# ccaven/tinyslam

Hardware: AMD Instinct MI355X
Metric: ORB extract throughput, 1280x720 (frames/sec; Mkeypoints/sec alongside) (higher is better)
Workload: dtype f32; 1 GPU; BASELINE.json configs[3]: batch of 256 independent 1280x720 RGBA frames per GPU, device-resident, full ORB (FAST-12 + orientation + blur + BRIEF-256); frames_per_gpu_per_batch=256, width=1280, height=720, hierarchy_depth=2, max_features=8192, content=default, mode=literal, input=rgba, pipeline=default, fp_contract=0, angle_bins=0, batches_in_flight=1, collate=none (1 GPU)

## Files before the change

tinyslam_amd/csrc/orb_api.hip:

```cpp
#include <hip/hip_runtime.h>
#include <chrono>
#include <cmath>

#include <cstdarg>
#include <cstdio>
#include <cstdlib>
#include <cstring>
#include <new>
#include <optional>
#include <string>
#include <algorithm>
#include <vector>

#include "../../include/tinyorb.h"
#include "orb_front_launch.h"
#include "orb_kernels_fused.h"
#include "orb_kernels_brief.h"
#include "orb_kernels_intended.h"
#include "orb_kernels_staged.h"
#include "orb_kernels_collate.h"
#include "orb_kernels_match.h"
#include "orb_kernels_verify.h"
#include "orb_kernels_epipolar.h"
#include "orb_kernels_guide.h"
// ... 146 lines not shown
    bool in_async[2] = {false, false};
    struct {
        bool single_memcpy = false, single_split = false, single_serial = false, single_sync = false, single_block = false;
        bool no_swizzle = false, quiet = false;
        bool front_generic = false, front_trace = false;
        int phase_mask = -1, brief_i_mask = -1, lds_pad = 0;
    } env;
    uint32_t* dv_count = nullptr;
    CornerData* dv_corners = nullptr;
    CornerDescriptor* dv_desc = nullptr;
    uint16_t* d_gray = nullptr;
    uint16_t* d_blur = nullptr;
    uint16_t* d_blur_rowc = nullptr;
    uint32_t blur_qa[kMaxLevels] = {0};
    uint32_t* d_counts = nullptr;
    CornerData* d_corners = nullptr;
    CornerDescriptor* d_desc = nullptr;
    uint32_t* out_counts[2] = {nullptr, nullptr};
    CornerData* out_corners[2] = {nullptr, nullptr};
    CornerDescriptor* out_desc[2] = {nullptr, nullptr};
    CornerData* d_seg = nullptr;
    uint32_t* d_seg_counts = nullptr;
    uint32_t* d_seg_before = nullptr;
    BandGeom bands{};
    RowsGeom rows{};
    BriefTGeom brieft{};
    bool use_brief_t = false;
    uint32_t band_rows_lvl[kMaxLevels] = {0};
    uint32_t ln_threads[kMaxLevels] = {0};
    uint32_t tile_w_lvl[kMaxLevels] = {0};
    uint32_t seg_classes = 1;
    uint32_t* d_pattern = nullptr;
    float* d_cos = nullptr;
    float* d_sin = nullptr;
    uint4* d_rot = nullptr;
    unsigned long long* d_stamps = nullptr;

    uint32_t* h_count = nullptr;
    uint32_t* d_single_done = nullptr;
    hipEvent_t single_done_ev = nullptr;
    uint32_t single_seq = 0;
    CornerData* h_corners = nullptr;
    CornerDescriptor* h_desc = nullptr;
    bool single_valid = false;

    uint32_t last_batch = 0;
// ... 375 lines not shown
}

bool brieft_geometry(const OrbProgram* p, const RowsGeom& rg, uint32_t n_classes, BriefTGeom* out) {
    BriefTGeom g{};
    g.n_slots = rg.n_slots;
    g.seg_cap = rg.seg_cap;
    g.n_classes = n_classes;
    uint32_t rows = 0;
    for (uint32_t m = 0; m < p->pyr.depth; m++) {
        g.flat_end[m] = rg.flat_end[m];
        g.qa[m] = rg.qa[m];
        g.row_base[m] = rows + (uint32_t)kBriefHalo;
        rows += p->pyr.h[m] + 2u * (uint32_t)kBriefHalo + 8u;
    }
    g.rows_padded = rows;
    g.oob = p->oob;
    *out = g;
    if (getenv("TINYORB_BRIEF_ROWS")) return false;
    return rg.n_slots >= 1u && rg.n_slots * n_classes <= kBriefTMaxSlots && rows <= kBriefTMaxRows;
}

int launch_brief(OrbProgram* p, hipStream_t s, uint32_t n, const RowsGeom& rows_geom, const uint16_t* d_blur,
                 const uint16_t* d_blur_rowc, const uint32_t* seg_counts, uint32_t* seg_before, const CornerData* seg,
                 uint32_t* d_counts, CornerData* d_corners, CornerDescriptor* d_desc) {
    const uint32_t cap = p->cfg.max_features;
    const BriefTables tab{p->d_pattern, p->d_cos, p->d_sin, p->d_rot};
    const bool use_t = p->use_brief_t;
    {
        LaunchScope ls(p, s, KID_PREFIX);
        hipLaunchKernelGGL(k_slot_prefix, dim3(n), dim3(64), 0, s, seg_counts, seg_before, d_counts, rows_geom.n_slots,
                           rows_geom.seg_cap, use_t ? p->brieft.n_classes : 1u);
    }
    if (use_t) {
        const BriefTGeom& tg = p->brieft;
        const dim3 grid(n, (cap + (uint32_t)kBriefNfChunk - 1u) / (uint32_t)kBriefNfChunk);
        {
            LaunchScope ls(p, s, KID_BRIEF_T);
#define BRIEF_T_LAUNCH(ROT_)                                                                                                         \
    hipLaunchKernelGGL((k_brief_t<kBriefTWaves, ROT_>), dim3(n, (cap + kBriefTThreads - 1u) / kBriefTThreads), dim3(kBriefTThreads), \
                       brieft_lds_bytes(tg), s, d_blur_rowc, p->pyr, tg, seg_counts, seg_before, seg, d_corners, cap, d_desc, tab)
            switch (rot_form(p->opt.fp_contract)) {
                case 1: BRIEF_T_LAUNCH(1); break;
                case 2: BRIEF_T_LAUNCH(2); break;
                default: BRIEF_T_LAUNCH(0); break;
            }
#undef BRIEF_T_LAUNCH
        }
        LaunchScope ls(p, s, KID_BRIEF_NF);
        if (p->oob != kOobZero)
            hipLaunchKernelGGL(k_brief_nf<true>, grid, dim3(256), 0, s, d_blur, d_blur_rowc, p->pyr, tg, seg_counts, seg_before, d_corners,
                               cap, d_desc, tab);
        else
            hipLaunchKernelGGL(k_brief_nf<false>, grid, dim3(256), 0, s, d_blur, d_blur_rowc, p->pyr, tg, seg_counts, seg_before, d_corners,
                               cap, d_desc, tab);
    } else {
        LaunchScope ls(p, s, KID_BRIEF_ROWS);
        RowsGeom rg = rows_geom;
        rg.oob = p->oob;
        rg.fp = p->opt.fp_contract;
        rg.split = 1u;
        while (rg.split < 16u && rg.n_slots * n * rg.split < 2048u) rg.split *= 2u;
        hipLaunchKernelGGL(k_brief_rows, dim3(rg.n_slots * rg.split, n), dim3(256), 0, s, d_blur, d_blur_rowc, p->pyr, rg,
                           seg_counts, seg_before, seg, d_corners, cap, d_desc, tab);
    }
    return ORB_OK;
}

FrontGeom fused_level_geometry(const OrbProgram* p, uint32_t lvl, uint32_t gw, uint32_t gh, uint32_t n) {
    const Pyramid& pyr = p->pyr;
    FrontGeom g = front_geometry(pyr, lvl, gw ? gw : 8u, gh, n, p->band_rows_lvl[lvl], p->tile_w_lvl[lvl], p->ln_threads[lvl]);
    if (gw == 0) g.gh = 0;
    g.slot_base = p->bands.slot_base[lvl];
    g.n_slots = p->bands.n_slots;
    g.seg_cap = p->bands.seg_cap;
    g.n_classes = p->seg_classes;
    g.stamps = p->d_stamps;
    if (p->env.phase_mask >= 0) g.phase_mask = (uint32_t)p->env.phase_mask;
// ... 51 lines not shown
            dim3 grid((pyr.w[lvl] + 63u) / 64u, (pyr.h[lvl] + 4u * kMipRows - 1u) / (4u * kMipRows), n);
            hipLaunchKernelGGL(k_mip, grid, dim3(64, 4), 0, sm, d_gray, pyr, lvl, (float)pyr.w[lvl - 1] / (float)pyr.w[lvl], (float)pyr.h[lvl - 1] / (float)pyr.h[lvl], p->wq);
        }
        const FrontGeom g = fused_level_geometry(p, lvl, gw, gh, n);
        hipStream_t s_lvl = s;
        if (g.n_bands * (g.tiled ? g.n_ct : 1u) != p->bands.slot_base[lvl + 1] - p->bands.slot_base[lvl])
            return fail(p, ORB_EINVAL, "internal: band count mismatch at level %u", lvl);
        if (!g.tiled && sizeof(BlurCol) * (size_t)g.n_var > 8u * (size_t)g.ts)
            return fail(p, ORB_EINVAL, "internal: blur column table of level %u does not fit", lvl);
        uint32_t lds = front_lds_bytes(g);
        lds += (uint32_t)p->env.lds_pad;
        if (lds > p->max_lds) return fail(p, ORB_EINVAL, "level %u needs %u bytes of LDS", lvl, lds);
        const dim3 grid(g.n_bands * (g.tiled ? g.n_ct : 1u) * n);
        FrontLaunch L{frames, p->frame_bytes, d_gray, d_blur, d_blur_rowc, pyr, g, p->threshold, d_seg_counts, d_seg, s_lvl, grid.x, lds,
                      p->band_rows_lvl[lvl], p->ln_threads[lvl], p->input_y8,
                      lvl == 0 && ((pyr.w[0] & 3u) || g.store_grey), p->oob != kOobZero, false};
        L.geo = front_pick_geo(p, L);
        {
            LaunchScope ls(p, s_lvl, lvl == 0 ? KID_FUSED_L0 : KID_FUSED_LN);
            const hipError_t e = kFrontLaunch[front_form(p->opt.fp_contract, lvl == 0 && !p->input_y8)](L);
            if (e != hipSuccess) return fail(p, ORB_EHIP, "k_front (level %u) failed to launch: %s", lvl, hipGetErrorString(e));
        }
    }
    if (with_brief) launch_brief(p, s, n, p->rows, d_blur, d_blur_rowc, d_seg_counts, d_seg_before, d_seg, d_counts, d_corners, d_desc);
    HIP_TRY(p, hipGetLastError());
    return ORB_OK;
}

int run_fused(OrbProgram* p, const uint8_t* frames, uint32_t n, hipStream_t s) {
    if (int rc = run_fused_range(p, frames, 0, n, s)) return rc;
    p->planes_valid = true;
    return ORB_OK;
}

uint32_t itile_width(uint32_t w) {
    const uint32_t w8 = (w + 7u) & ~7u;
    return w8 < (uint32_t)kITileW ? w8 : (uint32_t)kITileW;
}

bool fused_i_eligible(const OrbProgram* p) {
    if (!p->intended || (p->opt.flags & ORB_FLAG_STAGED)) return false;
    const Pyramid& pyr = p->pyr;
    if ((uint64_t)pyr.w[0] * pyr.h[0] > (1ull << 26)) return false;
    if ((pyr.w[0] & 3u) != 0u || pyr.w[0] < 8u) return false;
    return true;
}

// ... 514 lines not shown
    const size_t B = p->max_batch, cap = config->max_features;
    CREATE_TRY(hipMalloc(&p->d_gray, B * p->pyr.stride * sizeof(uint16_t)));
    CREATE_TRY(hipMalloc(&p->d_blur, B * p->pyr.stride * sizeof(uint16_t)));
    for (int set = 0; set < ((p->opt.flags & ORB_FLAG_DOUBLE_OUTPUT) ? 2 : 1); set++) {
        CREATE_TRY(hipMalloc(&p->out_counts[set], B * sizeof(uint32_t)));
        CREATE_TRY(hipMalloc(&p->out_corners[set], B * cap * sizeof(CornerData)));
        CREATE_TRY(hipMalloc(&p->out_desc[set], B * cap * sizeof(CornerDescriptor)));
        CREATE_TRY(hipMemset(p->out_counts[set], 0, B * sizeof(uint32_t)));
        CREATE_TRY(hipMemset(p->out_corners[set], 0, B * cap * sizeof(CornerData)));
        CREATE_TRY(hipMemset(p->out_desc[set], 0, B * cap * sizeof(CornerDescriptor)));
    }
    p->d_counts = p->out_counts[0];
    p->d_corners = p->out_corners[0];
    p->d_desc = p->out_desc[0];
    if (p->fused) {
        CREATE_TRY(hipMalloc(&p->d_blur_rowc, B * p->pyr.row_stride * sizeof(uint16_t)));
        CREATE_TRY(hipMemset(p->d_blur_rowc, 0, B * p->pyr.row_stride * sizeof(uint16_t)));
        const size_t lists = (size_t)p->bands.n_slots * p->seg_classes;
        CREATE_TRY(hipMalloc(&p->d_seg, B * lists * (size_t)p->bands.seg_cap * sizeof(CornerData)));
        CREATE_TRY(hipMalloc(&p->d_seg_counts, B * lists * sizeof(uint32_t)));
        CREATE_TRY(hipMemset(p->d_seg_counts, 0, B * lists * sizeof(uint32_t)));
        CREATE_TRY(hipMalloc(&p->d_seg_before, B * lists * sizeof(uint32_t)));
    }
    if (p->fused_x) {
        CREATE_TRY(hipMalloc(&p->d_blur_rowc, B * p->pyr.row_stride * sizeof(uint16_t)));
        CREATE_TRY(hipMemset(p->d_blur_rowc, 0, B * p->pyr.row_stride * sizeof(uint16_t)));
        CREATE_TRY(hipMalloc(&p->d_xband_counts, B * (size_t)p->xband_slots * sizeof(uint32_t)));
    }
    if (p->fused_i || p->fused_x) {
        const size_t n_seg = B * (size_t)p->itiles.n_slots;
        CREATE_TRY(hipMalloc(&p->d_iseg, n_seg * p->itiles.seg_cap * sizeof(CornerData)));
        CREATE_TRY(hipMalloc(&p->d_iseg_scores, n_seg * p->itiles.seg_cap * sizeof(float)));
        CREATE_TRY(hipMalloc(&p->d_iseg_counts, n_seg * sizeof(uint32_t)));
        CREATE_TRY(hipMemset(p->d_iseg_counts, 0, n_seg * sizeof(uint32_t)));
        CREATE_TRY(hipMalloc(&p->d_iseg_before, n_seg * sizeof(uint32_t)));
        CREATE_TRY(hipMalloc(&p->d_thr_key, B * sizeof(unsigned long long)));
    } else if (p->opt.flags & (ORB_FLAG_NMS | ORB_FLAG_INTENDED)) {
        uint32_t off = 0, width = W, height = H;
        for (uint32_t m = 0; m < p->pyr.depth; m++) {
            const uint32_t gw = ((width + 7u) / 8u) * 8u, gh = ((height + 7u) / 8u) * 8u;
            p->score_layout.off[m] = off;
            p->score_layout.pitch[m] = gw + 2u;
            off += (gw + 2u) * (gh + 2u);
            width /= 2u;
            height /= 2u;
        }
// ... 55 lines not shown
    if (!p) return;
    (void)hipSetDevice(p->device);
    if (p->stream) (void)hipStreamSynchronize(p->stream);
    for (auto& sp : p->pending) {
        (void)hipEventDestroy(sp.start);
        (void)hipEventDestroy(sp.stop);
    }
    for (auto e : p->event_pool) (void)hipEventDestroy(e);
    (void)hipFree(p->d_input);
    (void)hipFree(p->d_input_alt);
    for (hipEvent_t ev : p->in_uploaded)
        if (ev) (void)hipEventDestroy(ev);
    (void)hipFree(p->d_gray);
    (void)hipFree(p->d_blur);
    (void)hipFree(p->d_blur_rowc);
    for (int set = 0; set < 2; set++) {
        (void)hipFree(p->out_counts[set]);
        (void)hipFree(p->out_corners[set]);
        (void)hipFree(p->out_desc[set]);
    }
    (void)hipFree(p->d_seg);
    (void)hipFree(p->d_seg_counts);
    (void)hipFree(p->d_seg_before);
    (void)hipFree(p->d_score_planes);
    (void)hipFree(p->d_prov_counts);
    (void)hipFree(p->d_prov);
    (void)hipFree(p->d_prov_scores);
    (void)hipFree(p->d_xband_counts);
    (void)hipFree(p->d_iseg);
    (void)hipFree(p->d_iseg_scores);
    (void)hipFree(p->d_iseg_counts);
    (void)hipFree(p->d_iseg_before);
    (void)hipFree(p->d_thr_key);
    (void)hipFree(p->d_prov2_counts);
    (void)hipFree(p->d_prov2);
    (void)hipFree(p->d_prov2_scores);
    (void)hipFree(p->d_pattern);
    (void)hipFree(p->d_cos);
    (void)hipFree(p->d_sin);
    if (p->d_rot) (void)hipFree(p->d_rot);
    (void)hipFree(p->d_stamps);
    for (int st = 0; st < ST_COUNT; st++) {
        free_stage_buffers(p, st);
        if (p->stage[st].done) (void)hipEventDestroy(p->stage[st].done);
    }
    if (p->single_done_ev) (void)hipEventDestroy(p->single_done_ev);
// ... 1267 lines not shown
```

tinyslam_amd/csrc/orb_kernels_brief.h:

```cpp
#pragma once
#include "orb_kernels_fused.h"

namespace orb {

constexpr int kBriefTThreads = 256;
constexpr int kBriefTWaves = 6;
constexpr uint32_t kBriefTMaxSlots = 8192;
constexpr uint32_t kBriefTMaxRows = 12288;

struct BriefTGeom {
    uint32_t n_slots, seg_cap;
    uint32_t n_classes;
    uint32_t flat_end[kMaxLevels];
    uint32_t qa[kMaxLevels];
    uint32_t row_base[kMaxLevels];
    uint32_t rows_padded;
    uint32_t oob;
};

__host__ __device__ inline uint32_t brieft_lds_bytes(const BriefTGeom& g) {
    return (g.n_slots * g.n_classes + 1u) * 4u + ((g.rows_padded + 1u) & ~1u) * 2u;
}

__device__ __forceinline__ constexpr int pat_ax(int j) { return ORB_BRIEF_PATTERN[4 * j + 0]; }
__device__ __forceinline__ constexpr int pat_ay(int j) { return ORB_BRIEF_PATTERN[4 * j + 1]; }
__device__ __forceinline__ constexpr int pat_bx(int j) { return ORB_BRIEF_PATTERN[4 * j + 2]; }
__device__ __forceinline__ constexpr int pat_by(int j) { return ORB_BRIEF_PATTERN[4 * j + 3]; }

__device__ __forceinline__ uint32_t wave_inclusive_sum(uint32_t x) {
    int v = (int)x;
    v += __builtin_amdgcn_update_dpp(0, v, 0x111, 0xf, 0xf, true);
// ... 5 lines not shown
    return (uint32_t)v;
}

__device__ __forceinline__ void store_host_u32(uint32_t* p, uint32_t v) { *p = v; }
__device__ __forceinline__ void store_host_16(void* p, uint4 v) { *reinterpret_cast<uint4*>(p) = v; }

__device__ __forceinline__ uint32_t push_gt(uint32_t word, uint32_t a, uint32_t b) {
    return __builtin_amdgcn_alignbit(word, b - a, 31);
}

__device__ __forceinline__ void brief_t_stage_rows(uint16_t* rows, const uint16_t* __restrict__ src, const Pyramid& pyr,
                                                   const BriefTGeom& bg, uint32_t tid, uint32_t n_threads = kBriefTThreads) {
    uint32_t m = 0;
    for (uint32_t i = tid; i < bg.rows_padded; i += n_threads) {
        while (m + 1u < pyr.depth && i + (uint32_t)kBriefHalo >= bg.row_base[m + 1u]) m++;
        const uint32_t y = i - bg.row_base[m];
        uint16_t v = 0;
        if (y < pyr.h[m]) v = src[pyr.row_off[m] + y];
        else if (bg.oob != kOobZero) v = src[pyr.row_off[m] + (uint32_t)oob_index((int)y, (int)pyr.h[m], bg.oob)];
        rows[i] = v;
    }
}

template <int CHUNK = kBriefTThreads, bool STAGED = false, int ROT = 0>
__device__ __forceinline__ void brief_t_body(uint8_t* lds_raw, uint32_t frame, uint32_t chunk, const uint16_t* __restrict__ blur_rowc,
                                             const Pyramid& pyr, const BriefTGeom& bg, const uint32_t* __restrict__ seg_counts,
                                             const uint32_t* __restrict__ seg_before, const CornerData* __restrict__ segments,
                                             CornerData* __restrict__ corners, uint32_t cap,
                                             CornerDescriptor* __restrict__ descriptors, const BriefTables& tab,
                                             CornerData* __restrict__ host_corners = nullptr,
                                             CornerDescriptor* __restrict__ host_descriptors = nullptr) {
    const uint32_t n_ent = bg.n_slots * bg.n_classes;
    uint32_t* const before = reinterpret_cast<uint32_t*>(lds_raw);
    uint16_t* const rows = reinterpret_cast<uint16_t*>(before + n_ent + 1u);
    __shared__ uint32_t lv[kMaxLevels][2];

    const uint32_t tid = threadIdx.x;
    const size_t sbase = (size_t)frame * n_ent;
    uint32_t stored_total;
    if (STAGED) {
        if (tid < pyr.depth) lv[tid][0] = bg.flat_end[tid], lv[tid][1] = bg.row_base[tid];
        __syncthreads();
        stored_total = before[n_ent];
    } else {
        stored_total = seg_before[sbase + n_ent - 1u] + min(seg_counts[sbase + n_ent - 1u], bg.seg_cap);
    }
    const uint32_t n_frame = min(stored_total, cap);
    const uint32_t k0 = chunk * (uint32_t)CHUNK;
    if (k0 >= n_frame) return;

    if (!STAGED) {
        for (uint32_t s = tid; s < n_ent; s += kBriefTThreads) before[s] = seg_before[sbase + s];
        if (tid == 0) before[n_ent] = stored_total;
        if (tid < pyr.depth) lv[tid][0] = bg.flat_end[tid], lv[tid][1] = bg.row_base[tid];
        brief_t_stage_rows(rows, blur_rowc + (size_t)frame * pyr.row_stride, pyr, bg, tid);
        __syncthreads();
    }

    const uint32_t k = k0 + tid;
    if (tid >= (uint32_t)CHUNK || k >= n_frame) return;
    uint32_t lo = 0, hi = n_ent;
    while (hi - lo > 1u) {
        const uint32_t mid = (lo + hi) >> 1;
        if (before[mid] <= k)
            lo = mid;
        else
            hi = mid;
    }
    const uint32_t cls = lo >= bg.n_slots ? 1u : 0u, slot = lo - cls * bg.n_slots;
    const uint4 rec = *reinterpret_cast<const uint4*>(
        &segments[(((size_t)frame * bg.n_slots + slot) * bg.n_classes + cls) * bg.seg_cap + (k - before[lo])]);
    *reinterpret_cast<uint4*>(&corners[(size_t)frame * cap + k]) = rec;
    if (host_corners) store_host_16(&host_corners[k], rec);
    const uint32_t lvl = min(rec.w, pyr.depth - 1u);
    if (!(rec.x >= (uint32_t)kBriefHalo && rec.x < lv[lvl][0])) return;

    uint32_t d[8];
    uint4* const o = reinterpret_cast<uint4*>(descriptors + (size_t)frame * cap + k);
    if (bg.n_classes == 2u && k0 + (tid & ~63u) + 64u <= before[bg.n_slots]) {
        const uint16_t* base0 = rows + lv[lvl][1] + rec.y - kBriefHalo;
#pragma unroll
        for (int wd = 0; wd < 8; wd++) {
            uint32_t acc = 0;
#pragma unroll
            for (int i = 31; i >= 0; i--) {
                const int j = wd * 32 + i;
                acc = push_gt(acc, base0[pat_ay(j) + kBriefHalo], base0[pat_by(j) + kBriefHalo]);
            }
            d[wd] = acc;
        }
        o[0] = make_uint4(d[0], d[1], d[2], d[3]);
        o[1] = make_uint4(d[4], d[5], d[6], d[7]);
        if (host_descriptors) {
            store_host_16(reinterpret_cast<uint4*>(host_descriptors + k), make_uint4(d[0], d[1], d[2], d[3]));
            store_host_16(reinterpret_cast<uint4*>(host_descriptors + k) + 1, make_uint4(d[4], d[5], d[6], d[7]));
        }
        return;
    }
// ... 18 lines not shown
            } else {
                const float a2 = nstw * (float)pat_ax(j), a3 = ctw * (float)pat_ay(j);
                const float b2 = nstw * (float)pat_bx(j), b3 = ctw * (float)pat_by(j);
                ray = a2 + a3, rby = b2 + b3;
            }
            acc = push_gt(acc, base[(int)ray], base[(int)rby]);
        }
        d[wd] = acc;
    }
    o[0] = make_uint4(d[0], d[1], d[2], d[3]);
    o[1] = make_uint4(d[4], d[5], d[6], d[7]);
    if (host_descriptors) {
        store_host_16(reinterpret_cast<uint4*>(host_descriptors + k), make_uint4(d[0], d[1], d[2], d[3]));
        store_host_16(reinterpret_cast<uint4*>(host_descriptors + k) + 1, make_uint4(d[4], d[5], d[6], d[7]));
    }
}

template <int kWavesPerSimd, int ROT = 0>
__global__ __launch_bounds__(kBriefTThreads, kWavesPerSimd) void k_brief_t(const uint16_t* __restrict__ blur_rowc, Pyramid pyr, BriefTGeom bg,
                                                                const uint32_t* __restrict__ seg_counts,
                                                                const uint32_t* __restrict__ seg_before,
                                                                const CornerData* __restrict__ segments,
                                                                CornerData* __restrict__ corners, uint32_t cap,
                                                                CornerDescriptor* __restrict__ descriptors, BriefTables tab) {
    extern __shared__ __attribute__((aligned(16))) uint8_t lds_raw[];
    brief_t_body<kBriefTThreads, false, ROT>(lds_raw, blockIdx.x, blockIdx.y, blur_rowc, pyr, bg, seg_counts, seg_before, segments, corners, cap, descriptors, tab);
}

constexpr int kNfPatchCols = 48, kNfPatchRows = 2 * kBriefHalo + 1;
constexpr int kNfPatchHalfs = kNfPatchRows * kNfPatchCols;

__global__ __launch_bounds__(64) void k_rot_table(const uint32_t* __restrict__ pattern, const float* __restrict__ cos_tab,
                                                  const float* __restrict__ sin_tab, int pitch, int intended, uint4* __restrict__ out,
                                                  uint32_t fp = 0u, uint32_t angle_bins = 0u) {
    const uint32_t code = angle_bins ? (blockIdx.x * 6284u + 3142u) / angle_bins : blockIdx.x, lane = threadIdx.x;
    const float ct = cos_tab[code], st = sin_tab[code], nst = -st;
    uint32_t w[4];
#pragma unroll
    for (int e = 0; e < 4; e++) {
        const uint32_t pk = pattern[64u * (uint32_t)e + lane];
        const float pax = (float)(int8_t)(pk & 255u), pay = (float)(int8_t)((pk >> 8) & 255u);
        const float pbx = (float)(int8_t)((pk >> 16) & 255u), pby = (float)(int8_t)(pk >> 24);
        float rax, ray, rbx, rby;
        if (intended) {
            const float a0 = ct * pax, a1 = nst * pay, a2 = st * pax, a3 = ct * pay;
            const float b0 = ct * pbx, b1 = nst * pby, b2 = st * pbx, b3 = ct * pby;
            rax = a0 + a1, ray = a2 + a3, rbx = b0 + b1, rby = b2 + b3;
        } else {
            rotate_fp(ct, st, nst, pax, pay, rot_form(fp), &rax, &ray);
// ... 46 lines not shown
    __syncthreads();
    uint32_t start = 0, n_nf = 0;
#pragma unroll
    for (uint32_t w2 = 0; w2 < 4u; w2++) {
        if (w2 < wave) start += wave_n[w2];
        n_nf += wave_n[w2];
    }
    if (mine) list[start + (uint32_t)__popcll(m & ((1ull << lane) - 1ull))] = (uint16_t)tid;
    __syncthreads();
    if (wave >= n_nf) return;

    uint32_t* out_desc = reinterpret_cast<uint32_t*>(descriptors + (size_t)frame * cap + k0);
    uint16_t* const patch = patches[wave];
    for (uint32_t i = wave; i < n_nf; i += (uint32_t)NW) {
        const uint32_t idx = __builtin_amdgcn_readfirstlane((uint32_t)list[i]);
        uint4 r = recs[idx];
        r.x = __builtin_amdgcn_readfirstlane(r.x), r.y = __builtin_amdgcn_readfirstlane(r.y);
        r.z = __builtin_amdgcn_readfirstlane(r.z), r.w = __builtin_amdgcn_readfirstlane(r.w);
        const uint32_t lvl = min(r.w, pyr.depth - 1u);
        const int w = (int)__builtin_amdgcn_readfirstlane(lv[lvl][0]), h = (int)__builtin_amdgcn_readfirstlane(lv[lvl][1]);
        const int qa = (int)__builtin_amdgcn_readfirstlane(lv[lvl][2]);
        const uint16_t* rowc = blur_rowc + (size_t)frame * pyr.row_stride + __builtin_amdgcn_readfirstlane(lv[lvl][3]);
        const uint16_t* plane = blur + (size_t)frame * pyr.stride + __builtin_amdgcn_readfirstlane(lv[lvl][4]);
        const uint4 tt = tab.rot[(size_t)min(r.z, (uint32_t)(ORB_ANGLE_STEPS - 1)) * 64u + lane];
        const uint32_t tw[4] = {tt.x, tt.y, tt.z, tt.w};
        uint64_t bal[4];
        if ((w & 1) == 0) {
            const int c0 = ((int)r.x - kBriefHalo) & ~7;
            constexpr int kPiecesPerRow = kNfPatchCols / 8, kPieces = kNfPatchRows * kPiecesPerRow;
            constexpr int kRounds = (kPieces + 63) / 64;
            uint4 tv[kRounds];
            uint32_t rcv[kRounds];
            int kind[kRounds], where[kRounds];
#pragma unroll
            for (int rr = 0; rr < kRounds; rr++) {
                const int p = (int)lane + 64 * rr;
                const int pr = (int)(((float)p + 0.5f) * (1.0f / (float)kPiecesPerRow));
                const int pc = p - pr * kPiecesPerRow;
                const int gy0 = (int)r.y - kBriefHalo + pr, cx = c0 + 8 * pc;
                const int gy = OOB ? oob_index(gy0, h, bg.oob) : gy0;
                const bool in = p < kPieces && gy >= 0 && gy < h && cx >= 0 && cx < w;
                kind[rr] = !in ? 0 : (cx < qa ? 1 : (cx + 8 <= w ? 2 : 3));
                where[rr] = p < kPieces ? pr * kNfPatchCols + 8 * pc : -1;
                rcv[rr] = rowc[min(max(gy, 0), h - 1)];
                if (OOB && p < kPieces && !(cx >= 0 && cx < w)) {
                    const int xm = oob_index(cx, w, bg.oob);
                    if (xm >= qa) rcv[rr] = plane[(size_t)(uint32_t)(__mul24(gy, w) + xm)];
                    kind[rr] = 1;
                }
                tv[rr] = *reinterpret_cast<const uint4*>(plane + (kind[rr] == 2 ? (size_t)(uint32_t)(__mul24(gy, w) + cx) : (size_t)0));
            }
#pragma unroll
            for (int rr = 0; rr < kRounds; rr++) {
                uint4 v = make_uint4(0u, 0u, 0u, 0u);
                if (kind[rr] == 1) {
                    const uint32_t c2 = rcv[rr] | (rcv[rr] << 16);
                    v = make_uint4(c2, c2, c2, c2);
                } else if (kind[rr] == 2) {
                    v = tv[rr];
                } else if (kind[rr] == 3) {
                    const int p = (int)lane + 64 * rr;
                    const int pr = (int)(((float)p + 0.5f) * (1.0f / (float)kPiecesPerRow));
                    const int gy0 = (int)r.y - kBriefHalo + pr, cx = c0 + 8 * (p - pr * kPiecesPerRow);
                    const int gy = OOB ? oob_index(gy0, h, bg.oob) : gy0;
                    const uint16_t* src = plane + (size_t)(uint32_t)(__mul24(gy, w) + cx);
                    uint32_t t[8];
#pragma unroll
                    for (int q = 0; q < 8; q++) t[q] = cx + q < w ? (uint32_t)src[q] : (OOB ? (uint32_t)src[w - 1 - cx] : 0u);
                    v = make_uint4(t[0] | (t[1] << 16), t[2] | (t[3] << 16), t[4] | (t[5] << 16), t[6] | (t[7] << 16));
                }
                if (where[rr] >= 0) *reinterpret_cast<uint4*>(&patch[where[rr]]) = v;
            }
            __builtin_amdgcn_fence(__ATOMIC_RELEASE, "wavefront");
            __builtin_amdgcn_wave_barrier();
            const int xo = (int)r.x - c0;
            const uint8_t* const centre = reinterpret_cast<const uint8_t*>(patch + kBriefHalo * kNfPatchCols + xo);
#pragma unroll
            for (int e = 0; e < 4; e++) {
                const uint32_t va = *reinterpret_cast<const uint16_t*>(centre + rot_a(tw[e]));
                const uint32_t vb = *reinterpret_cast<const uint16_t*>(centre + rot_b(tw[e]));
                bal[e] = __ballot(va > vb);
            }
            __builtin_amdgcn_fence(__ATOMIC_RELEASE, "wavefront");
            __builtin_amdgcn_wave_barrier();
        } else {
            const int gy = (int)r.y - kBriefHalo + (int)lane;
            const uint32_t rowv = (gy >= 0 && gy < h && lane < 37u) ? (uint32_t)rowc[gy] : 0u;
#pragma unroll
            for (int e = 0; e < 4; e++) {
                const int oa = rot_a(tw[e]) >> 1, ob = rot_b(tw[e]) >> 1;
                const int dya = (oa + kNfPatchCols / 2 + 64 * kNfPatchCols) / kNfPatchCols - 64, dxa = oa - dya * kNfPatchCols;
                const int dyb = (ob + kNfPatchCols / 2 + 64 * kNfPatchCols) / kNfPatchCols - 64, dxb = ob - dyb * kNfPatchCols;
                const int xa = (int)r.x + dxa, ya = (int)r.y + dya;
                const int xb = (int)r.x + dxb, yb = (int)r.y + dyb;
                uint32_t va = (uint32_t)__shfl((int)rowv, dya + kBriefHalo);
                uint32_t vb = (uint32_t)__shfl((int)rowv, dyb + kBriefHalo);
                const bool ina = xa >= 0 && xa < w && ya >= 0 && ya < h;
                const bool inb = xb >= 0 && xb < w && yb >= 0 && yb < h;
                if (!ina)
                    va = OOB ? blur_sample_mapped(plane, rowc, w, h, qa, xa, ya, bg.oob) : 0u;
                else if (xa >= qa)
                    va = plane[(size_t)(uint32_t)(__mul24(ya, w) + xa)];
                if (!inb)
                    vb = OOB ? blur_sample_mapped(plane, rowc, w, h, qa, xb, yb, bg.oob) : 0u;
                else if (xb >= qa)
                    vb = plane[(size_t)(uint32_t)(__mul24(yb, w) + xb)];
                bal[e] = __ballot(va > vb);
            }
        }
        if (lane < 8u) {
            const uint64_t src = lane < 2u ? bal[0] : (lane < 4u ? bal[1] : (lane < 6u ? bal[2] : bal[3]));
            out_desc[(size_t)idx * 8u + lane] = (uint32_t)(src >> ((lane & 1u) * 32u));
            if (host_descriptors) store_host_u32(reinterpret_cast<uint32_t*>(host_descriptors + k0) + (size_t)idx * 8u + lane, (uint32_t)(src >> ((lane & 1u) * 32u)));
        }
    }
}

constexpr int kBriefNfChunk = 64;
template <bool OOB = false>
__global__ __launch_bounds__(256) void k_brief_nf(const uint16_t* __restrict__ blur, const uint16_t* __restrict__ blur_rowc,
                                                  Pyramid pyr, BriefTGeom bg, const uint32_t* __restrict__ seg_counts,
                                                  const uint32_t* __restrict__ seg_before,
                                                  const CornerData* __restrict__ corners, uint32_t cap,
                                                  CornerDescriptor* __restrict__ descriptors, BriefTables tab) {
    brief_nf_body<kBriefNfChunk, 4, OOB>(blockIdx.x, blockIdx.y, ~0u, blur, blur_rowc, pyr, bg, seg_counts, seg_before, corners, cap, descriptors, tab);
}

constexpr int kBriefOneChunk = 64;
constexpr int kSingleCountWords = 32, kSingleDoneWord = 16;
constexpr int kBriefOneThreads = 512;
template <int ROT = 0>
__global__ __launch_bounds__(kBriefOneThreads) void k_brief_one(const uint16_t* __restrict__ blur, const uint16_t* __restrict__ blur_rowc, Pyramid pyr,
                                                   BriefTGeom bg, const uint32_t* __restrict__ seg_counts,
                                                   uint32_t* __restrict__ seg_before, const CornerData* __restrict__ segments,
                                                   uint32_t* __restrict__ counts, CornerData* __restrict__ corners, uint32_t cap,
                                                   CornerDescriptor* __restrict__ descriptors, BriefTables tab,
                                                   uint32_t* __restrict__ host_count, CornerData* __restrict__ host_corners,
                                                   CornerDescriptor* __restrict__ host_descriptors, uint32_t* __restrict__ done_count,
                                                   uint32_t seq) {
    extern __shared__ __attribute__((aligned(16))) uint8_t lds_raw[];
    const uint32_t tid = threadIdx.x, chunk = blockIdx.x;
    const uint32_t n_ent = bg.n_slots * bg.n_classes;
#ifdef TINYORB_STAMPS
    uint64_t st[6];
    int n_st = 0;
#define BRIEF_ONE_STAMP() do { if (n_st < 6) st[n_st++] = wall_clock64(); } while (0)
#else
#define BRIEF_ONE_STAMP() do { } while (0)
// ... 60 lines not shown
```

Before: 544,900 frames/s.

## Pass non-flat keypoint bitmask from BRIEF-T kernel to skip empty NF blocks

The tiled BRIEF kernel now writes a per-64-keypoint ballot mask marking which keypoints fell outside the flat (row-cached) path. The follow-up non-flat BRIEF kernel reads this mask and exits immediately for chunks with no work, instead of recomputing segment prefix lookups and classifying every keypoint itself. It also specialises level-parameter lookup for two-level pyramids, avoiding the LDS table and barrier. This adds a small global mask buffer, an extra write per wave, and a dependency between the two kernels on the mask contents.

```diff
diff --git a/tinyslam_amd/csrc/orb_api.hip b/tinyslam_amd/csrc/orb_api.hip
--- a/tinyslam_amd/csrc/orb_api.hip
+++ b/tinyslam_amd/csrc/orb_api.hip
@@ -192,6 +192,7 @@
     CornerData* d_seg = nullptr;
     uint32_t* d_seg_counts = nullptr;
     uint32_t* d_seg_before = nullptr;
+    uint64_t* d_nf_mask[2] = {nullptr, nullptr};
     BandGeom bands{};
     RowsGeom rows{};
     BriefTGeom brieft{};
@@ -613,7 +614,7 @@
 
 int launch_brief(OrbProgram* p, hipStream_t s, uint32_t n, const RowsGeom& rows_geom, const uint16_t* d_blur,
                  const uint16_t* d_blur_rowc, const uint32_t* seg_counts, uint32_t* seg_before, const CornerData* seg,
-                 uint32_t* d_counts, CornerData* d_corners, CornerDescriptor* d_desc) {
+                 uint32_t* d_counts, CornerData* d_corners, CornerDescriptor* d_desc, uint32_t f0 = 0) {
     const uint32_t cap = p->cfg.max_features;
     const BriefTables tab{p->d_pattern, p->d_cos, p->d_sin, p->d_rot};
     const bool use_t = p->use_brief_t;
@@ -625,11 +626,13 @@
     if (use_t) {
         const BriefTGeom& tg = p->brieft;
         const dim3 grid(n, (cap + (uint32_t)kBriefNfChunk - 1u) / (uint32_t)kBriefNfChunk);
+        const uint32_t mask_words = brief_mask_words(cap);
+        uint64_t* const nf_mask = p->d_nf_mask[p->cur_set] + (size_t)f0 * mask_words;
         {
             LaunchScope ls(p, s, KID_BRIEF_T);
 #define BRIEF_T_LAUNCH(ROT_)                                                                                                         \
     hipLaunchKernelGGL((k_brief_t<kBriefTWaves, ROT_>), dim3(n, (cap + kBriefTThreads - 1u) / kBriefTThreads), dim3(kBriefTThreads), \
-                       brieft_lds_bytes(tg), s, d_blur_rowc, p->pyr, tg, seg_counts, seg_before, seg, d_corners, cap, d_desc, tab)
+                       brieft_lds_bytes(tg), s, d_blur_rowc, p->pyr, tg, seg_counts, seg_before, seg, d_corners, cap, d_desc, tab, nf_mask, mask_words)
             switch (rot_form(p->opt.fp_contract)) {
                 case 1: BRIEF_T_LAUNCH(1); break;
                 case 2: BRIEF_T_LAUNCH(2); break;
@@ -638,12 +641,16 @@
 #undef BRIEF_T_LAUNCH
         }
         LaunchScope ls(p, s, KID_BRIEF_NF);
-        if (p->oob != kOobZero)
-            hipLaunchKernelGGL(k_brief_nf<true>, grid, dim3(256), 0, s, d_blur, d_blur_rowc, p->pyr, tg, seg_counts, seg_before, d_corners,
-                               cap, d_desc, tab);
-        else
-            hipLaunchKernelGGL(k_brief_nf<false>, grid, dim3(256), 0, s, d_blur, d_blur_rowc, p->pyr, tg, seg_counts, seg_before, d_corners,
-                               cap, d_desc, tab);
+#define BRIEF_NF_LAUNCH(OOB_, TABLE_)                                                                                                  \
+    hipLaunchKernelGGL((k_brief_nf<OOB_, TABLE_>), grid, dim3(256), 0, s, d_blur, d_blur_rowc, p->pyr, tg, d_corners, cap, d_desc, tab, \
+                       nf_mask, mask_words)
+        const bool table = p->pyr.depth > 2u;
+        if (p->oob != kOobZero) {
+            if (table) BRIEF_NF_LAUNCH(true, true); else BRIEF_NF_LAUNCH(true, false);
+        } else {
+            if (table) BRIEF_NF_LAUNCH(false, true); else BRIEF_NF_LAUNCH(false, false);
+        }
+#undef BRIEF_NF_LAUNCH
     } else {
         LaunchScope ls(p, s, KID_BRIEF_ROWS);
         RowsGeom rg = rows_geom;
@@ -741,7 +748,7 @@
             if (e != hipSuccess) return fail(p, ORB_EHIP, "k_front (level %u) failed to launch: %s", lvl, hipGetErrorString(e));
         }
     }
-    if (with_brief) launch_brief(p, s, n, p->rows, d_blur, d_blur_rowc, d_seg_counts, d_seg_before, d_seg, d_counts, d_corners, d_desc);
+    if (with_brief) launch_brief(p, s, n, p->rows, d_blur, d_blur_rowc, d_seg_counts, d_seg_before, d_seg, d_counts, d_corners, d_desc, f0);
     HIP_TRY(p, hipGetLastError());
     return ORB_OK;
 }
@@ -1302,6 +1309,10 @@
         CREATE_TRY(hipMemset(p->d_seg_counts, 0, B * lists * sizeof(uint32_t)));
         CREATE_TRY(hipMalloc(&p->d_seg_before, B * lists * sizeof(uint32_t)));
     }
+    if (p->use_brief_t)
+        for (int set = 0; set < ((p->opt.flags & ORB_FLAG_DOUBLE_OUTPUT) ? 2 : 1); set++) {
+            CREATE_TRY(hipMalloc(&p->d_nf_mask[set], B * brief_mask_words((uint32_t)cap) * sizeof(uint64_t)));
+        }
     if (p->fused_x) {
         CREATE_TRY(hipMalloc(&p->d_blur_rowc, B * p->pyr.row_stride * sizeof(uint16_t)));
         CREATE_TRY(hipMemset(p->d_blur_rowc, 0, B * p->pyr.row_stride * sizeof(uint16_t)));
@@ -1403,6 +1414,7 @@
     (void)hipFree(p->d_seg);
     (void)hipFree(p->d_seg_counts);
     (void)hipFree(p->d_seg_before);
+    for (int set = 0; set < 2; set++) (void)hipFree(p->d_nf_mask[set]);
     (void)hipFree(p->d_score_planes);
     (void)hipFree(p->d_prov_counts);
     (void)hipFree(p->d_prov);
diff --git a/tinyslam_amd/csrc/orb_brief_nf_keypoint.inc b/tinyslam_amd/csrc/orb_brief_nf_keypoint.inc
--- /dev/null
+++ b/tinyslam_amd/csrc/orb_brief_nf_keypoint.inc
@@ -0,0 +1,91 @@
+        const uint4 tt = tab.rot[(size_t)min(r.z, (uint32_t)(ORB_ANGLE_STEPS - 1)) * 64u + lane];
+        const uint32_t tw[4] = {tt.x, tt.y, tt.z, tt.w};
+        uint64_t bal[4];
+        if ((w & 1) == 0) {
+            const int c0 = ((int)r.x - kBriefHalo) & ~7;
+            constexpr int kPiecesPerRow = kNfPatchCols / 8, kPieces = kNfPatchRows * kPiecesPerRow;
+            constexpr int kRounds = (kPieces + 63) / 64;
+            uint4 tv[kRounds];
+            uint32_t rcv[kRounds];
+            int kind[kRounds], where[kRounds];
+#pragma unroll
+            for (int rr = 0; rr < kRounds; rr++) {
+                const int p = (int)lane + 64 * rr;
+                const int pr = (int)(((float)p + 0.5f) * (1.0f / (float)kPiecesPerRow));
+                const int pc = p - pr * kPiecesPerRow;
+                const int gy0 = (int)r.y - kBriefHalo + pr, cx = c0 + 8 * pc;
+                const int gy = OOB ? oob_index(gy0, h, bg.oob) : gy0;
+                const bool in = p < kPieces && gy >= 0 && gy < h && cx >= 0 && cx < w;
+                kind[rr] = !in ? 0 : (cx < qa ? 1 : (cx + 8 <= w ? 2 : 3));
+                where[rr] = p < kPieces ? pr * kNfPatchCols + 8 * pc : -1;
+                rcv[rr] = rowc[min(max(gy, 0), h - 1)];
+                if (OOB && p < kPieces && !(cx >= 0 && cx < w)) {
+                    const int xm = oob_index(cx, w, bg.oob);
+                    if (xm >= qa) rcv[rr] = plane[(size_t)(uint32_t)(__mul24(gy, w) + xm)];
+                    kind[rr] = 1;
+                }
+                tv[rr] = *reinterpret_cast<const uint4*>(plane + (kind[rr] == 2 ? (size_t)(uint32_t)(__mul24(gy, w) + cx) : (size_t)0));
+            }
+#pragma unroll
+            for (int rr = 0; rr < kRounds; rr++) {
+                uint4 v = make_uint4(0u, 0u, 0u, 0u);
+                if (kind[rr] == 1) {
+                    const uint32_t c2 = rcv[rr] | (rcv[rr] << 16);
+                    v = make_uint4(c2, c2, c2, c2);
+                } else if (kind[rr] == 2) {
+                    v = tv[rr];
+                } else if (kind[rr] == 3) {
+                    const int p = (int)lane + 64 * rr;
+                    const int pr = (int)(((float)p + 0.5f) * (1.0f / (float)kPiecesPerRow));
+                    const int gy0 = (int)r.y - kBriefHalo + pr, cx = c0 + 8 * (p - pr * kPiecesPerRow);
+                    const int gy = OOB ? oob_index(gy0, h, bg.oob) : gy0;
+                    const uint16_t* src = plane + (size_t)(uint32_t)(__mul24(gy, w) + cx);
+                    uint32_t t[8];
+#pragma unroll
+                    for (int q = 0; q < 8; q++) t[q] = cx + q < w ? (uint32_t)src[q] : (OOB ? (uint32_t)src[w - 1 - cx] : 0u);
+                    v = make_uint4(t[0] | (t[1] << 16), t[2] | (t[3] << 16), t[4] | (t[5] << 16), t[6] | (t[7] << 16));
+                }
+                if (where[rr] >= 0) *reinterpret_cast<uint4*>(&patch[where[rr]]) = v;
+            }
+            __builtin_amdgcn_fence(__ATOMIC_RELEASE, "wavefront");
+            __builtin_amdgcn_wave_barrier();
+            const int xo = (int)r.x - c0;
+            const uint8_t* const centre = reinterpret_cast<const uint8_t*>(patch + kBriefHalo * kNfPatchCols + xo);
+#pragma unroll
+            for (int e = 0; e < 4; e++) {
+                const uint32_t va = *reinterpret_cast<const uint16_t*>(centre + rot_a(tw[e]));
+                const uint32_t vb = *reinterpret_cast<const uint16_t*>(centre + rot_b(tw[e]));
+                bal[e] = __ballot(va > vb);
+            }
+            __builtin_amdgcn_fence(__ATOMIC_RELEASE, "wavefront");
+            __builtin_amdgcn_wave_barrier();
+        } else {
+            const int gy = (int)r.y - kBriefHalo + (int)lane;
+            const uint32_t rowv = (gy >= 0 && gy < h && lane < 37u) ? (uint32_t)rowc[gy] : 0u;
+#pragma unroll
+            for (int e = 0; e < 4; e++) {
+                const int oa = rot_a(tw[e]) >> 1, ob = rot_b(tw[e]) >> 1;
+                const int dya = (oa + kNfPatchCols / 2 + 64 * kNfPatchCols) / kNfPatchCols - 64, dxa = oa - dya * kNfPatchCols;
+                const int dyb = (ob + kNfPatchCols / 2 + 64 * kNfPatchCols) / kNfPatchCols - 64, dxb = ob - dyb * kNfPatchCols;
+                const int xa = (int)r.x + dxa, ya = (int)r.y + dya;
+                const int xb = (int)r.x + dxb, yb = (int)r.y + dyb;
+                uint32_t va = (uint32_t)__shfl((int)rowv, dya + kBriefHalo);
+                uint32_t vb = (uint32_t)__shfl((int)rowv, dyb + kBriefHalo);
+                const bool ina = xa >= 0 && xa < w && ya >= 0 && ya < h;
+                const bool inb = xb >= 0 && xb < w && yb >= 0 && yb < h;
+                if (!ina)
+                    va = OOB ? blur_sample_mapped(plane, rowc, w, h, qa, xa, ya, bg.oob) : 0u;
+                else if (xa >= qa)
+                    va = plane[(size_t)(uint32_t)(__mul24(ya, w) + xa)];
+                if (!inb)
+                    vb = OOB ? blur_sample_mapped(plane, rowc, w, h, qa, xb, yb, bg.oob) : 0u;
+                else if (xb >= qa)
+                    vb = plane[(size_t)(uint32_t)(__mul24(yb, w) + xb)];
+                bal[e] = __ballot(va > vb);
+            }
+        }
+        if (lane < 8u) {
+            const uint64_t src = lane < 2u ? bal[0] : (lane < 4u ? bal[1] : (lane < 6u ? bal[2] : bal[3]));
+            out_desc[(size_t)idx * 8u + lane] = (uint32_t)(src >> ((lane & 1u) * 32u));
+            if (host_descriptors) store_host_u32(reinterpret_cast<uint32_t*>(host_descriptors + k0) + (size_t)idx * 8u + lane, (uint32_t)(src >> ((lane & 1u) * 32u)));
+        }
diff --git a/tinyslam_amd/csrc/orb_kernels_brief.h b/tinyslam_amd/csrc/orb_kernels_brief.h
--- a/tinyslam_amd/csrc/orb_kernels_brief.h
+++ b/tinyslam_amd/csrc/orb_kernels_brief.h
@@ -7,6 +7,7 @@
 constexpr int kBriefTWaves = 6;
 constexpr uint32_t kBriefTMaxSlots = 8192;
 constexpr uint32_t kBriefTMaxRows = 12288;
+__host__ __device__ inline uint32_t brief_mask_words(uint32_t cap) { return 4u * ((cap + (uint32_t)kBriefTThreads - 1u) / (uint32_t)kBriefTThreads); }
 
 struct BriefTGeom {
     uint32_t n_slots, seg_cap;
@@ -58,14 +59,16 @@
     }
 }
 
-template <int CHUNK = kBriefTThreads, bool STAGED = false, int ROT = 0>
+template <int CHUNK = kBriefTThreads, bool STAGED = false, int ROT = 0, bool MASK = false>
 __device__ __forceinline__ void brief_t_body(uint8_t* lds_raw, uint32_t frame, uint32_t chunk, const uint16_t* __restrict__ blur_rowc,
                                              const Pyramid& pyr, const BriefTGeom& bg, const uint32_t* __restrict__ seg_counts,
                                              const uint32_t* __restrict__ seg_before, const CornerData* __restrict__ segments,
                                              CornerData* __restrict__ corners, uint32_t cap,
                                              CornerDescriptor* __restrict__ descriptors, const BriefTables& tab,
                                              CornerData* __restrict__ host_corners = nullptr,
-                                             CornerDescriptor* __restrict__ host_descriptors = nullptr) {
+                                             CornerDescriptor* __restrict__ host_descriptors = nullptr,
+                                             uint64_t* __restrict__ nf_mask = nullptr, uint32_t mask_words = 0) {
+    static_assert(!MASK || (CHUNK == kBriefTThreads && !STAGED), "the mask is the batch kernel's: 256 keypoints, four words");
     const uint32_t n_ent = bg.n_slots * bg.n_classes;
     uint32_t* const before = reinterpret_cast<uint32_t*>(lds_raw);
     uint16_t* const rows = reinterpret_cast<uint16_t*>(before + n_ent + 1u);
@@ -83,7 +86,11 @@
     }
     const uint32_t n_frame = min(stored_total, cap);
     const uint32_t k0 = chunk * (uint32_t)CHUNK;
-    if (k0 >= n_frame) return;
+    uint64_t* const mask_word = MASK ? nf_mask + (size_t)frame * mask_words + (k0 >> 6) + (tid >> 6) : nullptr;
+    if (k0 >= n_frame) {
+        if (MASK && (tid & 63u) == 0u) *mask_word = 0ull;
+        return;
+    }
 
     if (!STAGED) {
         for (uint32_t s = tid; s < n_ent; s += kBriefTThreads) before[s] = seg_before[sbase + s];
@@ -94,22 +101,34 @@
     }
 
     const uint32_t k = k0 + tid;
-    if (tid >= (uint32_t)CHUNK || k >= n_frame) return;
-    uint32_t lo = 0, hi = n_ent;
-    while (hi - lo > 1u) {
-        const uint32_t mid = (lo + hi) >> 1;
-        if (before[mid] <= k)
-            lo = mid;
-        else
-            hi = mid;
-    }
-    const uint32_t cls = lo >= bg.n_slots ? 1u : 0u, slot = lo - cls * bg.n_slots;
-    const uint4 rec = *reinterpret_cast<const uint4*>(
-        &segments[(((size_t)frame * bg.n_slots + slot) * bg.n_classes + cls) * bg.seg_cap + (k - before[lo])]);
-    *reinterpret_cast<uint4*>(&corners[(size_t)frame * cap + k]) = rec;
-    if (host_corners) store_host_16(&host_corners[k], rec);
+    const bool live = k < n_frame;
+    if (!MASK && (tid >= (uint32_t)CHUNK || !live)) return;
+    uint4 fetched = make_uint4(0u, 0u, 0u, 0u);
+    if (!MASK || live) {
+        uint32_t lo = 0, hi = n_ent;
+        while (hi - lo > 1u) {
+            const uint32_t mid = (lo + hi) >> 1;
+            if (before[mid] <= k)
+                lo = mid;
+            else
+                hi = mid;
+        }
+        const uint32_t cls = lo >= bg.n_slots ? 1u : 0u, slot = lo - cls * bg.n_slots;
+        fetched = *reinterpret_cast<const uint4*>(
+            &segments[(((size_t)frame * bg.n_slots + slot) * bg.n_classes + cls) * bg.seg_cap + (k - before[lo])]);
+        *reinterpret_cast<uint4*>(&corners[(size_t)frame * cap + k]) = fetched;
+        if (host_corners) store_host_16(&host_corners[k], fetched);
+    }
+    const uint4 rec = fetched;
     const uint32_t lvl = min(rec.w, pyr.depth - 1u);
-    if (!(rec.x >= (uint32_t)kBriefHalo && rec.x < lv[lvl][0])) return;
+    if constexpr (MASK) {
+        const bool flat = live && rec.x >= (uint32_t)kBriefHalo && rec.x < lv[lvl][0];
+        const uint64_t not_flat = __ballot(live && !flat);
+        if ((tid & 63u) == 0u) *mask_word = not_flat;
+        if (!flat) return;
+    } else {
+        if (!(rec.x >= (uint32_t)kBriefHalo && rec.x < lv[lvl][0])) return;
+    }
 
     uint32_t d[8];
     uint4* const o = reinterpret_cast<uint4*>(descriptors + (size_t)frame * cap + k);
@@ -174,9 +193,11 @@
                                                                 const uint32_t* __restrict__ seg_before,
                                                                 const CornerData* __restrict__ segments,
                                                                 CornerData* __restrict__ corners, uint32_t cap,
-                                                                CornerDescriptor* __restrict__ descriptors, BriefTables tab) {
+                                                                CornerDescriptor* __restrict__ descriptors, BriefTables tab,
+                                                                uint64_t* __restrict__ nf_mask, uint32_t mask_words) {
     extern __shared__ __attribute__((aligned(16))) uint8_t lds_raw[];
-    brief_t_body<kBriefTThreads, false, ROT>(lds_raw, blockIdx.x, blockIdx.y, blur_rowc, pyr, bg, seg_counts, seg_before, segments, corners, cap, descriptors, tab);
+    brief_t_body<kBriefTThreads, false, ROT, true>(lds_raw, blockIdx.x, blockIdx.y, blur_rowc, pyr, bg, seg_counts, seg_before, segments, corners, cap, descriptors, tab,
+                                                   nullptr, nullptr, nf_mask, mask_words);
 }
 
 constexpr int kNfPatchCols = 48, kNfPatchRows = 2 * kBriefHalo + 1;
@@ -269,108 +290,71 @@
         const int qa = (int)__builtin_amdgcn_readfirstlane(lv[lvl][2]);
         const uint16_t* rowc = blur_rowc + (size_t)frame * pyr.row_stride + __builtin_amdgcn_readfirstlane(lv[lvl][3]);
         const uint16_t* plane = blur + (size_t)frame * pyr.stride + __builtin_amdgcn_readfirstlane(lv[lvl][4]);
-        const uint4 tt = tab.rot[(size_t)min(r.z, (uint32_t)(ORB_ANGLE_STEPS - 1)) * 64u + lane];
-        const uint32_t tw[4] = {tt.x, tt.y, tt.z, tt.w};
-        uint64_t bal[4];
-        if ((w & 1) == 0) {
-            const int c0 = ((int)r.x - kBriefHalo) & ~7;
-            constexpr int kPiecesPerRow = kNfPatchCols / 8, kPieces = kNfPatchRows * kPiecesPerRow;
-            constexpr int kRounds = (kPieces + 63) / 64;
-            uint4 tv[kRounds];
-            uint32_t rcv[kRounds];
-            int kind[kRounds], where[kRounds];
-#pragma unroll
-            for (int rr = 0; rr < kRounds; rr++) {
-                const int p = (int)lane + 64 * rr;
-                const int pr = (int)(((float)p + 0.5f) * (1.0f / (float)kPiecesPerRow));
-                const int pc = p - pr * kPiecesPerRow;
-                const int gy0 = (int)r.y - kBriefHalo + pr, cx = c0 + 8 * pc;
-                const int gy = OOB ? oob_index(gy0, h, bg.oob) : gy0;
-                const bool in = p < kPieces && gy >= 0 && gy < h && cx >= 0 && cx < w;
-                kind[rr] = !in ? 0 : (cx < qa ? 1 : (cx + 8 <= w ? 2 : 3));
-                where[rr] = p < kPieces ? pr * kNfPatchCols + 8 * pc : -1;
-                rcv[rr] = rowc[min(max(gy, 0), h - 1)];
-                if (OOB && p < kPieces && !(cx >= 0 && cx < w)) {
-                    const int xm = oob_index(cx, w, bg.oob);
-                    if (xm >= qa) rcv[rr] = plane[(size_t)(uint32_t)(__mul24(gy, w) + xm)];
-                    kind[rr] = 1;
-                }
-                tv[rr] = *reinterpret_cast<const uint4*>(plane + (kind[rr] == 2 ? (size_t)(uint32_t)(__mul24(gy, w) + cx) : (size_t)0));
-            }
-#pragma unroll
-            for (int rr = 0; rr < kRounds; rr++) {
-                uint4 v = make_uint4(0u, 0u, 0u, 0u);
-                if (kind[rr] == 1) {
-                    const uint32_t c2 = rcv[rr] | (rcv[rr] << 16);
-                    v = make_uint4(c2, c2, c2, c2);
-                } else if (kind[rr] == 2) {
-                    v = tv[rr];
-                } else if (kind[rr] == 3) {
-                    const int p = (int)lane + 64 * rr;
-                    const int pr = (int)(((float)p + 0.5f) * (1.0f / (float)kPiecesPerRow));
-                    const int gy0 = (int)r.y - kBriefHalo + pr, cx = c0 + 8 * (p - pr * kPiecesPerRow);
-                    const int gy = OOB ? oob_index(gy0, h, bg.oob) : gy0;
-                    const uint16_t* src = plane + (size_t)(uint32_t)(__mul24(gy, w) + cx);
-                    uint32_t t[8];
-#pragma unroll
-                    for (int q = 0; q < 8; q++) t[q] = cx + q < w ? (uint32_t)src[q] : (OOB ? (uint32_t)src[w - 1 - cx] : 0u);
-                    v = make_uint4(t[0] | (t[1] << 16), t[2] | (t[3] << 16), t[4] | (t[5] << 16), t[6] | (t[7] << 16));
-                }
-                if (where[rr] >= 0) *reinterpret_cast<uint4*>(&patch[where[rr]]) = v;
-            }
-            __builtin_amdgcn_fence(__ATOMIC_RELEASE, "wavefront");
-            __builtin_amdgcn_wave_barrier();
-            const int xo = (int)r.x - c0;
-            const uint8_t* const centre = reinterpret_cast<const uint8_t*>(patch + kBriefHalo * kNfPatchCols + xo);
-#pragma unroll
-            for (int e = 0; e < 4; e++) {
-                const uint32_t va = *reinterpret_cast<const uint16_t*>(centre + rot_a(tw[e]));
-                const uint32_t vb = *reinterpret_cast<const uint16_t*>(centre + rot_b(tw[e]));
-                bal[e] = __ballot(va > vb);
-            }
-            __builtin_amdgcn_fence(__ATOMIC_RELEASE, "wavefront");
-            __builtin_amdgcn_wave_barrier();
+#include "orb_brief_nf_keypoint.inc"
+    }
+}
+
+constexpr int kBriefNfChunk = 64;
+template <bool OOB = false, bool TABLE = false>
+__device__ __forceinline__ void brief_nf_mask_body(uint32_t frame, uint32_t chunk, const uint16_t* __restrict__ blur,
+                                                   const uint16_t* __restrict__ blur_rowc, const Pyramid& pyr, const BriefTGeom& bg,
+                                                   const CornerData* __restrict__ corners, uint32_t cap,
+                                                   CornerDescriptor* __restrict__ descriptors, const BriefTables& tab,
+                                                   const uint64_t* __restrict__ nf_mask, uint32_t mask_words) {
+    constexpr int NW = 4;
+    __shared__ __attribute__((aligned(16))) uint16_t patches[NW][kNfPatchHalfs];
+    __shared__ uint32_t lv[kMaxLevels][5];
+    CornerDescriptor* const host_descriptors = nullptr;
+    const uint32_t tid = threadIdx.x, lane = tid & 63u, wave = __builtin_amdgcn_readfirstlane(tid >> 6);
+    const uint32_t k0 = chunk * (uint32_t)kBriefNfChunk;
+    const uint64_t m = nf_mask[(size_t)frame * mask_words + chunk];
+    if (m == 0ull) return;
+    if constexpr (TABLE) {
+        if (tid < pyr.depth) {
+            lv[tid][0] = pyr.w[tid], lv[tid][1] = pyr.h[tid], lv[tid][2] = bg.qa[tid], lv[tid][3] = pyr.row_off[tid];
+            lv[tid][4] = pyr.off[tid];
+        }
+        __syncthreads();
+    }
+    const uint32_t rank = __builtin_amdgcn_mbcnt_hi((uint32_t)(m >> 32), __builtin_amdgcn_mbcnt_lo((uint32_t)m, 0u));
+    const bool mine = ((m >> lane) & 1ull) != 0ull && rank % (uint32_t)NW == wave;
+    uint64_t left = __ballot(mine);
+    if (left == 0ull) return;
+    uint4 rec = make_uint4(0u, 0u, 0u, 0u);
+    if (mine) rec = *reinterpret_cast<const uint4*>(&corners[(size_t)frame * cap + k0 + lane]);
+
+    uint32_t* out_desc = reinterpret_cast<uint32_t*>(descriptors + (size_t)frame * cap + k0);
+    uint16_t* const patch = patches[wave];
+    do {
+        const uint32_t idx = (uint32_t)__builtin_ctzll(left);
+        left &= left - 1ull;
+        uint4 r;
+        r.x = (uint32_t)__builtin_amdgcn_readlane((int)rec.x, (int)idx), r.y = (uint32_t)__builtin_amdgcn_readlane((int)rec.y, (int)idx);
+        r.z = (uint32_t)__builtin_amdgcn_readlane((int)rec.z, (int)idx), r.w = (uint32_t)__builtin_amdgcn_readlane((int)rec.w, (int)idx);
+        const uint32_t lvl = min(r.w, pyr.depth - 1u);
+        int w, h, qa;
+        const uint16_t *rowc, *plane;
+        if constexpr (TABLE) {
+            w = (int)__builtin_amdgcn_readfirstlane(lv[lvl][0]), h = (int)__builtin_amdgcn_readfirstlane(lv[lvl][1]);
+            qa = (int)__builtin_amdgcn_readfirstlane(lv[lvl][2]);
+            rowc = blur_rowc + (size_t)frame * pyr.row_stride + __builtin_amdgcn_readfirstlane(lv[lvl][3]);
+            plane = blur + (size_t)frame * pyr.stride + __builtin_amdgcn_readfirstlane(lv[lvl][4]);
         } else {
-            const int gy = (int)r.y - kBriefHalo + (int)lane;
-            const uint32_t rowv = (gy >= 0 && gy < h && lane < 37u) ? (uint32_t)rowc[gy] : 0u;
-#pragma unroll
-            for (int e = 0; e < 4; e++) {
-                const int oa = rot_a(tw[e]) >> 1, ob = rot_b(tw[e]) >> 1;
-                const int dya = (oa + kNfPatchCols / 2 + 64 * kNfPatchCols) / kNfPatchCols - 64, dxa = oa - dya * kNfPatchCols;
-                const int dyb = (ob + kNfPatchCols / 2 + 64 * kNfPatchCols) / kNfPatchCols - 64, dxb = ob - dyb * kNfPatchCols;
-                const int xa = (int)r.x + dxa, ya = (int)r.y + dya;
-                const int xb = (int)r.x + dxb, yb = (int)r.y + dyb;
-                uint32_t va = (uint32_t)__shfl((int)rowv, dya + kBriefHalo);
-                uint32_t vb = (uint32_t)__shfl((int)rowv, dyb + kBriefHalo);
-                const bool ina = xa >= 0 && xa < w && ya >= 0 && ya < h;
-                const bool inb = xb >= 0 && xb < w && yb >= 0 && yb < h;
-                if (!ina)
-                    va = OOB ? blur_sample_mapped(plane, rowc, w, h, qa, xa, ya, bg.oob) : 0u;
-                else if (xa >= qa)
-                    va = plane[(size_t)(uint32_t)(__mul24(ya, w) + xa)];
-                if (!inb)
-                    vb = OOB ? blur_sample_mapped(plane, rowc, w, h, qa, xb, yb, bg.oob) : 0u;
-                else if (xb >= qa)
-                    vb = plane[(size_t)(uint32_t)(__mul24(yb, w) + xb)];
-                bal[e] = __ballot(va > vb);
-            }
-        }
-        if (lane < 8u) {
-            const uint64_t src = lane < 2u ? bal[0] : (lane < 4u ? bal[1] : (lane < 6u ? bal[2] : bal[3]));
-            out_desc[(size_t)idx * 8u + lane] = (uint32_t)(src >> ((lane & 1u) * 32u));
-            if (host_descriptors) store_host_u32(reinterpret_cast<uint32_t*>(host_descriptors + k0) + (size_t)idx * 8u + lane, (uint32_t)(src >> ((lane & 1u) * 32u)));
-        }
-    }
-}
-
-constexpr int kBriefNfChunk = 64;
-template <bool OOB = false>
+            const bool up = lvl != 0u;
+            w = (int)(up ? pyr.w[1] : pyr.w[0]), h = (int)(up ? pyr.h[1] : pyr.h[0]), qa = (int)(up ? bg.qa[1] : bg.qa[0]);
+            rowc = blur_rowc + (size_t)frame * pyr.row_stride + (up ? pyr.row_off[1] : pyr.row_off[0]);
+            plane = blur + (size_t)frame * pyr.stride + (up ? pyr.off[1] : pyr.off[0]);
+        }
+#include "orb_brief_nf_keypoint.inc"
+    } while (left != 0ull);
+}
+
+template <bool OOB = false, bool TABLE = false>
 __global__ __launch_bounds__(256) void k_brief_nf(const uint16_t* __restrict__ blur, const uint16_t* __restrict__ blur_rowc,
-                                                  Pyramid pyr, BriefTGeom bg, const uint32_t* __restrict__ seg_counts,
-                                                  const uint32_t* __restrict__ seg_before,
-                                                  const CornerData* __restrict__ corners, uint32_t cap,
-                                                  CornerDescriptor* __restrict__ descriptors, BriefTables tab) {
-    brief_nf_body<kBriefNfChunk, 4, OOB>(blockIdx.x, blockIdx.y, ~0u, blur, blur_rowc, pyr, bg, seg_counts, seg_before, corners, cap, descriptors, tab);
+                                                  Pyramid pyr, BriefTGeom bg, const CornerData* __restrict__ corners, uint32_t cap,
+                                                  CornerDescriptor* __restrict__ descriptors, BriefTables tab,
+                                                  const uint64_t* __restrict__ nf_mask, uint32_t mask_words) {
+    brief_nf_mask_body<OOB, TABLE>(blockIdx.x, blockIdx.y, blur, blur_rowc, pyr, bg, corners, cap, descriptors, tab, nf_mask, mask_words);
 }
 
 constexpr int kBriefOneChunk = 64;
```

Result: faster. 551,500 frames/s (median of 6 runs) (+1.2%).
